# lfalive/fast-genomic-data-processing

Hardware: AMD Instinct MI355X
Metric: PairHMM GCUPS (higher is better)
Workload: dtype f32

## Files before the change

### fast-genomic-data-processing_amd/csrc/mgx_pairhmm.hip

```cpp
#include <hip/hip_runtime.h>

#include <algorithm>
#include <atomic>
#include <cerrno>
#include <cmath>
#include <cstdarg>
#include <cstdio>
#include <cstdlib>
#include <cstring>
#include <chrono>
#include <memory>
#include <mutex>
#include <new>
#include <thread>
#include <string>
#include <vector>

#include "../../include/mgx_pairhmm.h"
#include "mgx_common.h"
#include "mgx_tables.h"
#include "pairhmm_pack.h"
#include "pairhmm_kernels.hip.inc"

using mgx::set_error;
// ... 2 lines not shown

constexpr int kNarrowMaxRPL = 8, kG8MaxRPL = 8, kG16MaxRPL = 12, kG64MinRPL = 4, kG64MaxRPL = 16;
constexpr int kMaxRowsG4 = 4 * kNarrowMaxRPL, kMaxRowsG8 = 8 * kG8MaxRPL;
constexpr int kMaxRowsG16 = 16 * kG16MaxRPL;
constexpr int kMaxRowsG64 = 64 * kG64MaxRPL;
constexpr int kMaxRowsStrip = 1 << 20;
constexpr int kStripMarkRPL = kG64MaxRPL + 1;
constexpr uint32_t kMaxLdsPerBlock = 64 * 1024;

struct Bin {
    int G = 0, RPL = 0;
    int Gd = 0, RPLd = 0;
    uint32_t job_begin = 0, job_count = 0;
    uint32_t max_h = 0;
    uint64_t cells = 0, alg_bytes = 0;
    uint32_t block = 256, lds_stride = 0, grid_f32 = 0, grid_f64 = 0, grid_f64_all = 0;
    bool strip = false;
};


struct Slab {
    uint8_t* dev = nullptr;
    uint8_t* pin = nullptr;
    size_t cap = 0, pin_cap = 0;
};
constexpr size_t kStageLimit = 256u << 20;
constexpr size_t kMaxEventSets = 64;
constexpr size_t kMinSlab = 1u << 20;
}

struct mgx_pairhmm {
// ... 10 lines not shown
    int n_cu = 256;
    std::vector<Slab> free_slabs;
    void* d_strip = nullptr; size_t strip_cap = 0;
};

struct mgx_pairhmm_batch {
    uint64_t n_pairs = 0;
    std::vector<Bin> bins;
    Slab slab;
    size_t in_bytes = 0, o_out = 0, o_used = 0, result_bytes = 0;
    uint8_t *d_bases = nullptr, *d_qual = nullptr, *d_ins = nullptr, *d_del = nullptr,
            *d_gcp = nullptr, *d_hap = nullptr, *d_used = nullptr;
    Job* d_jobs = nullptr;
    uint32_t* d_rerun_list = nullptr;
    uint32_t* d_rerun_count = nullptr;
    double* d_out = nullptr;
    std::vector<Job> host_jobs;
    bool has_model = false;
    uint32_t n_reads = 0;
    uint64_t* d_read_len = nullptr;
    uint8_t* d_keep = nullptr;
    uint32_t *d_row_off = nullptr, *d_row_nh = nullptr;
    size_t o_keep = 0;
    double log10_rate = 0, max_err = 0;
    hipEvent_t uploaded = nullptr;
    std::vector<hipEvent_t> ev;
    std::vector<uint64_t> acct_cells, acct_bytes;
    std::vector<int8_t> acct_multi;
    uint32_t ev_sets = 0;
    uint32_t runs_timed = 0;
// ... 26 lines not shown
    HIP_TRY(hipMalloc((void**)dst, bytes));
    if (src) HIP_TRY(hipMemcpyAsync(*dst, src, bytes, hipMemcpyHostToDevice, s));
    return 0;
}

inline void shape_of(uint32_t R, int* G, int* RPL) {
    static const int min_g = [] { const char* e = getenv("MGX_PAIRHMM_MIN_G"); const int v = e ? atoi(e) : 4; return v; }();
    const uint32_t g8_rows = (uint32_t)kMaxRowsG8;
    if (R <= (uint32_t)kMaxRowsG4 && min_g <= 4) { *G = 4; *RPL = (int)((R + 3) / 4); }
    else if (R <= g8_rows && min_g <= 8) { *G = 8; *RPL = (int)((R + 7) / 8); }
    else if (R <= (uint32_t)kMaxRowsG16) { *G = 16; *RPL = (int)((R + 15) / 16); }
    else if (R <= (uint32_t)kMaxRowsG64) { *G = 64; *RPL = std::max(kG64MinRPL, (int)((R + 63) / 64)); }
    else if (R <= (uint32_t)kMaxRowsStrip) { *G = 64; *RPL = kStripMarkRPL; }
    else { *G = 0; *RPL = 0; }
}
inline uint32_t lds_bytes(const Bin& bin, bool f32) {
    const uint32_t waves = bin.block / 64u, groups = bin.block / (uint32_t)(f32 ? bin.G : bin.Gd);
    const uint32_t etab = f32 ? (uint32_t)((bin.RPL + 1) / 2) * kNumCodes * 512u : 0u;
    return waves * etab + groups * bin.lds_stride;
}
constexpr int kBinG8 = kNarrowMaxRPL, kBinG16 = kBinG8 + kG8MaxRPL, kBinG64 = kBinG16 + kG16MaxRPL;
constexpr int kBinStrip = kBinG64 + (kG64MaxRPL - kG64MinRPL + 1);
constexpr int kBins = kBinStrip + 1;
inline int bin_index(int G, int RPL) {
    if (G == 64 && RPL == kStripMarkRPL) return kBinStrip;
    return G == 4 ? RPL - 1 : G == 8 ? kBinG8 + RPL - 1 : G == 16 ? kBinG16 + RPL - 1 : kBinG64 + RPL - kG64MinRPL;
}
inline void bin_shape(int k, Bin* b) {
    if (k == kBinStrip) { b->G = 64; b->RPL = kG64MaxRPL; b->Gd = 64; b->RPLd = kG64MaxRPL; b->strip = true; return; }
    if (k < kBinG8) { b->G = 4; b->RPL = k + 1; }
    else if (k < kBinG16) { b->G = 8; b->RPL = k - kBinG8 + 1; }
    else if (k < kBinG64) { b->G = 16; b->RPL = k - kBinG16 + 1; }
    else { b->G = 64; b->RPL = k - kBinG64 + kG64MinRPL; }
    if (b->G == 16 && b->RPL > 8) { b->Gd = 64; b->RPLd = (16 * b->RPL + 63) / 64; }
    else { b->Gd = b->G; b->RPLd = b->RPL; }
}
constexpr uint64_t kMergeBelow = 4096;

int finalize_bin(Bin& bin, int n_cu) {
    bin.lds_stride = (bin.max_h + 2u * (uint32_t)std::max(bin.G, bin.Gd) + 8u + 15u) & ~15u;
    bin.block = 64;
    if (const char* e = getenv("MGX_PAIRHMM_BLOCK")) { const int v = atoi(e); if (v == 64 || v == 128 || v == 256) bin.block = (uint32_t)v; }
    while (bin.block > 64u && lds_bytes(bin, true) > kMaxLdsPerBlock) bin.block /= 2;
    if (lds_bytes(bin, true) > 160u * 1024u) {
        set_error("haplotype of %u bases does not fit the LDS staging buffer", bin.max_h);
        return -E2BIG;
    }
    if (bin.strip) {
        bin.block = 64;
        bin.grid_f32 = bin.grid_f64 = bin.grid_f64_all = std::min<uint32_t>(bin.job_count, (uint32_t)n_cu * 4u);
        return 0;
    }
    const uint32_t gpb = bin.block / bin.G, gpbd = bin.block / bin.Gd;
    bin.grid_f32 = (bin.job_count + gpb - 1) / gpb;
    bin.grid_f64_all = (bin.job_count + gpbd - 1) / gpbd;
    bin.grid_f64 = std::min<uint32_t>(bin.grid_f64_all, (uint32_t)n_cu * 8u);
    return 0;
}
void merge_small_bins(uint64_t (&count)[kBins], int (&remap)[kBins]) {
    for (int k = 0; k < kBins; ++k) remap[k] = k;
    for (int k = 0; k + 1 < kBins; ++k) {
        if (k + 1 == kBinG8 || k + 1 == kBinG16 || k + 1 == kBinG64 || k + 1 == kBinStrip) continue;
        if (count[k] && count[k] < kMergeBelow) { count[k + 1] += count[k]; count[k] = 0; remap[k] = k + 1; }
    }
    for (int k = 0; k < kBins; ++k) { int t = k; while (remap[t] != t) t = remap[t]; remap[k] = t; }
}

inline size_t align_up(size_t x, size_t a = 256) { return (x + a - 1) / a * a; }

int acquire_slab(mgx_pairhmm* c, size_t bytes, size_t pin_bytes, Slab* out) {
    int best = -1;
// ... 137 lines not shown
    release_slab(c, b->slab);
    if (b->uploaded) (void)hipEventDestroy(b->uploaded);
    if (b->done) (void)hipEventDestroy(b->done);
    for (auto e : b->ev) (void)hipEventDestroy(e);
    delete b;
}

namespace {

struct SlabLayout {
    uint64_t n = 0, n_reads = 0, n_haps = 0, n_regions = 0, read_bytes = 0, hap_bytes = 0;
    bool cross = false, model = false;
    size_t rtab = 0, rreg = 0, rpre = 0, gtab = 0, htab = 0;
    size_t jobs = 0, bases = 0, qual = 0, ins = 0, del = 0, gcp = 0, hap = 0;
    size_t mapq = 0, rlen = 0, roff = 0, rnh = 0;
    size_t rlist = 0, rcount = 0;
    size_t pin_bytes = 0;
    bool staged = true;
};

int lay_out_slab(mgx_pairhmm* c, bool always_stage, SlabLayout* L, mgx_pairhmm_batch* b) {
    size_t off = 0;
    auto take = [&off](size_t bytes) { const size_t at = off; off = align_up(off + bytes); return at; };
    const uint64_t n = L->n, per_read = L->model ? L->n_reads : 0;
    if (L->cross) {
        L->rtab = take(L->n_reads * sizeof(SeqRef));
        L->rreg = take(L->n_reads * sizeof(uint32_t));
        L->rpre = take((L->n_reads + 1) * sizeof(uint32_t));
        L->gtab = take(L->n_regions * sizeof(RegionRef));
        L->htab = take(L->n_haps * sizeof(SeqRef));
    } else {
// ... 5 lines not shown
    L->del = take(L->read_bytes);
    L->gcp = take(L->read_bytes);
    L->hap = take(L->hap_bytes);
    L->mapq = take(per_read);
    L->rlen = take(per_read * sizeof(uint64_t));
    L->roff = take(per_read * sizeof(uint32_t));
    L->rnh = take(per_read * sizeof(uint32_t));
    b->in_bytes = off;
    b->o_out = take(n * sizeof(double));
    b->o_used = take(n);
    b->o_keep = take(per_read);
    b->result_bytes = off - b->o_out;
    L->pin_bytes = off;
    if (L->cross) L->jobs = take(n * sizeof(Job));
    L->rlist = take(2 * n * sizeof(uint32_t));
    L->rcount = take(64 * sizeof(uint32_t));
    L->staged = always_stage || L->pin_bytes <= kStageLimit;
    if (const int rc = acquire_slab(c, off, L->staged ? L->pin_bytes : 0, &b->slab)) return rc;
    uint8_t* dv = b->slab.dev;
    b->d_jobs = (Job*)(dv + L->jobs);
    b->d_bases = dv + L->bases; b->d_qual = dv + L->qual; b->d_ins = dv + L->ins; b->d_del = dv + L->del;
    b->d_gcp = dv + L->gcp; b->d_hap = dv + L->hap;
    b->d_out = (double*)(dv + b->o_out); b->d_used = dv + b->o_used;
    b->d_rerun_list = (uint32_t*)(dv + L->rlist); b->d_rerun_count = (uint32_t*)(dv + L->rcount);
    if (L->model) {
        b->d_read_len = (uint64_t*)(dv + L->rlen); b->d_keep = dv + b->o_keep;
        b->d_row_off = (uint32_t*)(dv + L->roff); b->d_row_nh = (uint32_t*)(dv + L->rnh);
    }
    return 0;
}

ReadModel make_read_model(const mgx_read_model_t& model) {
    ReadModel rm{};
    rm.rate_factor = model.pcr_rate_factor; rm.bq_threshold = model.base_quality_threshold;
    rm.constant_gcp = model.constant_gcp;
    for (int i = 0; i <= 20; ++i) {
        const double d = 40.0 - std::exp((double)i / ((double)std::max(rm.rate_factor, 1) * M_PI));
        const int v = (d > 0.0 ? (int)(d + 0.5) : (int)(d - 0.5)) + 1;
        rm.pcr_cache[i] = (uint8_t)(char)std::max(10, v);
// ... 349 lines not shown
    mgx_pairhmm_batch* b = r.b;
    if (!r.timing) return 0;
    if (b->ev.empty()) {
        const size_t per = b->bins.size() * 4;
        b->ev_sets = (uint32_t)std::max<size_t>(1, std::min<size_t>(kMaxEventSets, 1024 / per));
        b->ev.resize(per * b->ev_sets);
        for (auto& e : b->ev) HIP_TRY(hipEventCreate(&e));
    }
    r.ev = b->ev.data() + (size_t)(b->runs_timed % b->ev_sets) * b->bins.size() * 4;
    return 0;
}

int begin_run(Run& r) {
    mgx_pairhmm* c = r.c; mgx_pairhmm_batch* b = r.b;
    if (b->uploaded) HIP_TRY(hipStreamWaitEvent(r.s, b->uploaded, 0));
    HIP_TRY(hipMemsetAsync(b->d_rerun_count, 0, 64 * sizeof(uint32_t), r.s));
    HIP_TRY(hipMemsetAsync(b->d_used, 0, b->n_pairs, r.s));
    r.n_str = (int)std::min<size_t>((size_t)c->n_streams, b->bins.size());
    if (r.n_str > 1) {
        HIP_TRY(hipEventRecord(c->ev_fork, r.s));
        for (int q = 0; q + 1 < r.n_str; ++q) HIP_TRY(hipStreamWaitEvent(c->aux[q], c->ev_fork, 0));
    }
    KernelArgs& base = r.base;
    base.jobs = b->d_jobs;
    base.bases = b->d_bases; base.qual = b->d_qual; base.ins = b->d_ins; base.del = b->d_del;
    base.gcp = b->d_gcp; base.hap_bases = b->d_hap;
    base.out_log10 = b->d_out; base.used_f64 = b->d_used;
    base.log10_initial_f = c->log10_initial_f;
    base.log10_initial_d = c->log10_initial_d;
    return 0;
}

void survey_narrow(Run& r) {
    const std::vector<Bin>& bins = r.b->bins;
    r.first_narrow = bins.size();
    for (size_t k = 0; k < bins.size(); ++k) {
        const Bin& bn = bins[k];
        if (!is_narrow(bn)) continue;
        if (r.first_narrow == bins.size()) r.first_narrow = k;
        r.n_narrow_jobs = std::max(r.n_narrow_jobs, bn.job_begin + bn.job_count);
        r.narrow_max_h = std::max(r.narrow_max_h, bn.max_h);
        r.narrow_rows = std::max(r.narrow_rows, (uint32_t)(bn.G * bn.RPL));
// ... 17 lines not shown
        return bx.RPL != by.RPL ? bx.RPL > by.RPL : bx.G > by.G;
    });
    MultiArgs m{};
    m.a = r.base;
    m.a.rerun_list = b->d_rerun_list; m.a.rerun_count = b->d_rerun_count + kSharedCount;
    m.a.job_list = nullptr; m.a.n_dyn = nullptr;
    m.a.ph2pr = c->d_ph2pr_f; m.a.mm = c->d_mm_f; m.a.ph2pr_div3 = c->d_div3_f; m.a.gap_ratio = c->d_ratio_f;
    m.n_bins = (uint32_t)set.size();
    uint32_t blocks = 0, lds = 0;
    size_t book = set[0];
    uint64_t cells = 0, bytes = 0;
    for (size_t q = 0; q < set.size(); ++q) {
        const Bin& bn = b->bins[set[q]];
        m.block_first[q] = blocks; blocks += bn.grid_f32;
        m.job_first[q] = bn.job_begin; m.job_count[q] = bn.job_count; m.lds_stride[q] = bn.lds_stride;
        m.G[q] = (uint8_t)bn.G; m.RPL[q] = (uint8_t)bn.RPL;
        lds = std::max(lds, lds_bytes(bn, true));
        if (bn.cells > b->bins[book].cells) book = set[q];
        cells += bn.cells; bytes += bn.alg_bytes;
        r.in_multi[set[q]] = 1;
        b->acct_cells[set[q]] = 0; b->acct_bytes[set[q]] = 0;
    }
    m.block_first[set.size()] = blocks;
    b->acct_cells[book] = cells; b->acct_bytes[book] = bytes; b->acct_multi[book] = (int8_t)(1 + gset);
    if (r.timing) for (size_t q : set) if (q != book) { HIP_TRY(hipEventRecord(r.ev[4 * q + 0], r.s)); HIP_TRY(hipEventRecord(r.ev[4 * q + 1], r.s)); }
    if (r.timing) HIP_TRY(hipEventRecord(r.ev[4 * book + 0], r.s));
    if (gset == 0) hipLaunchKernelGGL(pairhmm_fwd_multi<0>, dim3(blocks), dim3(64), lds, r.s, m);
    else           hipLaunchKernelGGL(pairhmm_fwd_multi<1>, dim3(blocks), dim3(64), lds, r.s, m);
    if (r.timing) HIP_TRY(hipEventRecord(r.ev[4 * book + 1], r.s));
    return 0;
}

// ... 20 lines not shown
int launch_class(Run& r, size_t k, hipStream_t sk) {
    mgx_pairhmm* c = r.c; mgx_pairhmm_batch* b = r.b;
    hipEvent_t* ev = r.ev;
    const Bin& bin = b->bins[k];
    const bool shared = is_narrow(bin) && !r.force_f64;
    KernelArgs a = r.base;
    if (bin.strip) {
        a.strip_stride = (bin.max_h + 63u) & ~63u;
        if (const int rc = ensure_strip_scratch(c, (size_t)bin.grid_f32 * 6u * a.strip_stride * sizeof(double))) return rc;
        a.strip_scratch = c->d_strip;
    }
    a.rerun_list = shared ? b->d_rerun_list : b->d_rerun_list + bin.job_begin;
    a.rerun_count = b->d_rerun_count + (shared ? kSharedCount : (int)k);
    a.lds_stride = bin.lds_stride;
    a.job_first = bin.job_begin;
    if (!r.force_f64 && !r.in_multi[k]) {
        a.job_list = nullptr; a.n_dyn = nullptr; a.n_static = bin.job_count;
        a.ph2pr = c->d_ph2pr_f; a.mm = c->d_mm_f; a.ph2pr_div3 = c->d_div3_f; a.gap_ratio = c->d_ratio_f;
        KernelFn f = bin.strip ? (KernelFn)pairhmm_fwd_strip<float> : pick_kernel<float>(bin.G, bin.RPL);
        if (!f) { set_error("no fp32 kernel for G=%d RPL=%d", bin.G, bin.RPL); return -ENOSYS; }
        if (r.timing) HIP_TRY(hipEventRecord(ev[4 * k + 0], sk));
        hipLaunchKernelGGL(f, dim3(bin.grid_f32), dim3(bin.block), lds_bytes(bin, true), sk, a);
        if (r.timing) HIP_TRY(hipEventRecord(ev[4 * k + 1], sk));
    }
    const bool books_shared = shared && k == r.first_narrow;
    if (r.timing && !books_shared) HIP_TRY(hipEventRecord(ev[4 * k + 2], sk));
    if (!shared) {
        if (r.force_f64) { a.job_list = nullptr; a.n_dyn = nullptr; a.n_static = bin.job_count; }
        else { a.job_list = a.rerun_list; a.n_dyn = a.rerun_count; a.n_static = 0; }
        const int rc = launch_f64(r, a, bin.Gd, bin.RPLd, r.force_f64 ? bin.grid_f64_all : bin.grid_f64, bin.block, lds_bytes(bin, false), sk);
        if (rc) return rc;
    }
    if (r.timing && !books_shared) HIP_TRY(hipEventRecord(ev[4 * k + 3], sk));
    return 0;
}

int launch_classes(Run& r) {
    mgx_pairhmm* c = r.c; mgx_pairhmm_batch* b = r.b;
    std::vector<size_t> order(b->bins.size());
    for (size_t k = 0; k < order.size(); ++k) order[k] = k;
    std::stable_sort(order.begin(), order.end(), [&](size_t x, size_t y) { return b->bins[x].cells > b->bins[y].cells; });
    for (size_t at = 0; at < order.size(); ++at) {
        hipStream_t sk = (int)(at % (size_t)r.n_str) == 0 ? r.s : c->aux[at % (size_t)r.n_str - 1];
        if (const int rc = launch_class(r, order[at], sk)) return rc;
    }
    for (int q = 0; q + 1 < r.n_str; ++q) {
        HIP_TRY(hipEventRecord(c->ev_join[q], c->aux[q]));
        HIP_TRY(hipStreamWaitEvent(r.s, c->ev_join[q], 0));
    }
    return 0;
}

int launch_shared_f64(Run& r) {
    if (!r.n_narrow_jobs || r.force_f64) return 0;
    KernelArgs a = r.base;
    a.job_list = r.b->d_rerun_list; a.n_dyn = r.b->d_rerun_count + kSharedCount; a.n_static = 0; a.job_first = 0;
    a.lds_stride = (r.narrow_max_h + 2u * 16u + 8u + 15u) & ~15u;
    const int RPLd = (int)((r.narrow_rows + 15) / 16);
// ... 60 lines not shown
    if (!c) { set_error("ctx is NULL"); return -EINVAL; }
    HIP_TRY(hipSetDevice(c->device));
    HIP_TRY(hipStreamSynchronize(c->compute));
    return 0;
}

int mgx_pairhmm_batch_stats(mgx_pairhmm_t* c, mgx_pairhmm_batch_t* b, mgx_pairhmm_stats_t* out) {
    if (!c || !b || !out) { set_error("NULL argument"); return -EINVAL; }
    HIP_TRY(hipSetDevice(c->device));
    HIP_TRY(hipStreamSynchronize(c->compute));
    mgx_pairhmm_stats_t st = b->stats;
    const bool force_f64 = (c->flags & MGX_PAIRHMM_FORCE_DOUBLE) != 0;
    st.n_launches_f32 = force_f64 ? 0 : (uint32_t)b->bins.size();
    st.n_launches_f64 = (uint32_t)b->bins.size();
    st.n_rerun_f64 = 0;
    if (b->ran && b->n_pairs) {
        std::vector<uint32_t> cnt(64);
        HIP_TRY(hipMemcpy(cnt.data(), b->d_rerun_count, 64 * sizeof(uint32_t), hipMemcpyDeviceToHost));
        for (size_t k = 0; k < b->bins.size(); ++k) st.n_rerun_f64 += force_f64 ? b->bins[k].job_count : cnt[k];
        if (!force_f64) st.n_rerun_f64 += cnt[63];
        st.n_exact = cnt[62];
    }
    st.ms_f32 = st.ms_f64 = st.ms_f32_dominant = 0;
    st.dominant_cells = st.dominant_alg_bytes = 0;
    st.dominant_kernel[0] = 0;
    st.n_runs_timed = 0;
    if ((c->flags & MGX_PAIRHMM_TIMING) && b->ran && !b->ev.empty() && b->runs_timed) {
        const uint32_t n_sets = std::min(b->runs_timed, b->ev_sets);
        const bool acct = b->acct_cells.size() == b->bins.size();
        auto cells_of = [&](size_t k) { return acct ? b->acct_cells[k] : b->bins[k].cells; };
        size_t dom = 0;
        for (size_t k = 0; k < b->bins.size(); ++k) if (cells_of(k) >= cells_of(dom)) dom = k;
        double f32 = 0, f64 = 0, domms = 0;
// ... 387 lines not shown
```

### fast-genomic-data-processing_amd/csrc/pairhmm_kernels.hip.inc

```

#include <type_traits>

namespace {

struct Job {
    uint64_t read_off;
    uint64_t hap_off;
    uint32_t R;
    uint32_t H;
    uint32_t pair;
    uint32_t pad_;
};
static_assert(sizeof(Job) == 32, "Job is 32 bytes");

struct KernelArgs {
    const Job* jobs;
    const uint32_t* job_list;
    const uint32_t* n_dyn;
    uint32_t n_static;
    uint32_t job_first;
    const uint8_t* bases;
    const uint8_t* qual;
    const uint8_t* ins;
    const uint8_t* del;
    const uint8_t* gcp;
    const uint8_t* hap_bases;
    const void* ph2pr;
    const void* mm;
    const void* ph2pr_div3;
    const void* gap_ratio;
    double* out_log10;
    uint8_t* used_f64;
    uint32_t* rerun_list;
    uint32_t* rerun_count;
    uint32_t lds_stride;
    void* strip_scratch;
    uint32_t strip_stride;
    float log10_initial_f;
    double log10_initial_d;
};

constexpr double kExactBelow = 1e-280;
constexpr int kCodeN = 4;
constexpr int kCodePad = 7;

__device__ __forceinline__ int base_code(int b) {
    int c = 0;
    c = (b == 'C') ? 1 : c;
    c = (b == 'T') ? 2 : c;
// ... 41 lines not shown
    const int src = (j == G - 1) ? lane : lane + S;
    return __shfl(v, src, 64);
}

__device__ __forceinline__ float fma_(float a, float b, float c) { return __builtin_fmaf(a, b, c); }
__device__ __forceinline__ double fma_(double a, double b, double c) { return __builtin_fma(a, b, c); }

template <typename T> struct Prec;
template <> struct Prec<float> {
    static __device__ __forceinline__ float initial() { return 0x1p120f; }
};
template <> struct Prec<double> {
    static __device__ __forceinline__ double initial() { return 0x1p1020; }
};

#ifndef MGX_PAIRHMM_CODES
#define MGX_PAIRHMM_CODES 5
#endif
constexpr int kNumCodes = MGX_PAIRHMM_CODES;
template <int RPL> constexpr int etab_bytes_per_wave() { return ((RPL + 1) / 2) * kNumCodes * 64 * 8; }

template <typename T, int G, int RPL, bool STRIP = false, bool EXACT = false>
__device__ __forceinline__ void pairhmm_body(const KernelArgs& a, uint8_t* smem, const uint32_t block, const uint32_t n_blocks) {
    constexpr int GPW = 64 / G;
    constexpr bool kETab = (sizeof(T) == 4);
    constexpr bool kSix = (sizeof(T) == 4) && !EXACT;
    constexpr int RP2 = (RPL + 1) / 2;
    constexpr int S = lane_stride<G>();
    const int gpb = (int)blockDim.x / G;
    const int tid = (int)threadIdx.x;
    const int lane = tid & 63;
    const int wave = tid >> 6;
    const int j = G < 16 ? (lane & 15) / S : lane % G;
    const int grp = wave * GPW + (G < 16 ? (lane >> 4) * S + (lane & 15) % S : lane / G);
    const int n_waves = (int)blockDim.x >> 6;
    uint8_t* etab = smem + (kETab ? (size_t)wave * etab_bytes_per_wave<RPL>() : 0);
    uint8_t* hapbuf = smem + (kETab ? (size_t)n_waves * etab_bytes_per_wave<RPL>() : 0) +
                      (size_t)grp * a.lds_stride;
    const T* __restrict__ ph2pr = (const T*)a.ph2pr;
    const T* __restrict__ mm = (const T*)a.mm;
    const T* __restrict__ ph2pr_div3 = (const T*)a.ph2pr_div3;
    const T* __restrict__ gap_ratio = (const T*)a.gap_ratio;
    const uint32_t n_jobs = a.n_dyn ? *a.n_dyn : a.n_static;

    for (uint32_t base = block * (uint32_t)gpb; base < n_jobs; base += n_blocks * (uint32_t)gpb) {
        const uint32_t slot = base + (uint32_t)grp;
        const bool live = slot < n_jobs;
        uint32_t job_idx = 0;
        Job job;
        job.read_off = 0; job.hap_off = 0; job.R = 0; job.H = 0; job.pair = 0; job.pad_ = 0;
        if (live) {
            job_idx = a.job_list ? a.job_list[slot] : a.job_first + slot;
// ... 95 lines not shown
                    rb[s] = code;
                }
            }
        }
        if constexpr (kETab) {
            float* et = reinterpret_cast<float*>(etab) + lane * 2;
#pragma unroll
            for (int s = 0; s < RPL; ++s)
#pragma unroll
                for (int code = 0; code < kNumCodes; ++code)
                    et[((s >> 1) * kNumCodes + code) * 128 + (s & 1)] =
                        (code == rb[s] || code == kCodeN) ? eM[s] : eX[s];
        }
        __syncthreads();

        const int nsteps_g = live ? (H + nl - 1) : 0;
        int nmax = nsteps_g, nmin = live ? nsteps_g : 0x7fffffff;
        if constexpr (GPW > 1) {
#pragma unroll
            for (int off = 1; off < 64; off <<= 1) {
                if (off >= S && off < (G < 16 ? 16 : G)) continue;
                const int o1 = __shfl_xor(nmax, off, 64), o2 = __shfl_xor(nmin, off, 64);
                nmax = o1 > nmax ? o1 : nmax;
                nmin = o2 < nmin ? o2 : nmin;
            }
        }
        nmax = __builtin_amdgcn_readfirstlane(nmax);
        nmin = __builtin_amdgcn_readfirstlane(nmin);
        if (nmin > nmax) nmin = nmax;

        const uint8_t* hp_lane = hapbuf + (G - j);
        const uint8_t* et_lane = etab + lane * 8;
// ... 63 lines not shown
                }
                y_above = SIX ? init_y : g_own[0] * init_y;
            }
            const T old_y = (j == 0) ? y_above : (T)0;
            T uaM = 0, uaX = 0, uaY = old_y, ubM = 0, ubX = 0, ubY = old_y;
            if constexpr (STRIP) {
                if (strip > 0) {
                    uaY = 0; ubY = 0;
                    if (j == 0 && H > 0) { ubM = bprev[0]; ubX = bprev[a.strip_stride]; ubY = bprev[2u * a.strip_stride]; }
                }
            }

            auto column = [&](const T (&ec)[RPL], T& o2M, T& o2X, T& o2Y, const T o1M, const T o1X, bool count, const int dcol) {
                T Mn[RPL], Xn[RPL], Yn[RPL];
                if constexpr (SIX) {
                    Mn[0] = fma_(k3[0], o2Y, fma_(o2M, k0[0], o2X)) * ec[0];
                    Xn[0] = fma_(o1X, k2[0], o1M * k1[0]);
                    Yn[0] = fma_(py[0], k4[0], pm[0]);
#pragma unroll
                    for (int s = 1; s < RPL; ++s) {
                        Mn[s] = fma_(k3[s], py[s - 1], fma_(pm[s - 1], k0[s], px[s - 1])) * ec[s];
                        Xn[s] = fma_(Xn[s - 1], k2[s], Mn[s - 1] * k1[s]);
                        Yn[s] = fma_(py[s], k4[s], pm[s]);
                    }
                } else if constexpr (SC) {
                    Mn[0] = (fma_(o2M, k0[0], o2X) + o2Y) * ec[0];
                    Xn[0] = fma_(o1X, k2[0], o1M * k1[0]);
                    Yn[0] = fma_(py[0], k4[0], pm[0] * k3[0]);
#pragma unroll
                    for (int s = 1; s < RPL; ++s) {
                        Mn[s] = (fma_(pm[s - 1], k0[s], px[s - 1]) + py[s - 1]) * ec[s];
                        Xn[s] = fma_(Xn[s - 1], k2[s], Mn[s - 1] * k1[s]);
                        Yn[s] = fma_(py[s], k4[s], pm[s] * k3[s]);
                    }
                } else if constexpr (EXACT) {
                    Mn[0] = ((o2M * k0[0] + o2X * k1[0]) + o2Y * k1[0]) * ec[0];
                    Xn[0] = o1M * k2[0] + o1X * k3[0];
                    Yn[0] = pm[0] * k4[0] + py[0] * k3[0];
#pragma unroll
// ... 52 lines not shown
                t = uaM; uaM = ubM; ubM = t;
                t = uaX; uaX = ubX; ubX = t;
                t = uaY; uaY = ubY; ubY = t;
                load_e(hn, e);
            }
        };
        if constexpr (EXACT) sweep(std::integral_constant<int, kPlain>{});
        else if (use_plain) sweep(std::integral_constant<int, kPlain>{});
        else if constexpr (kSix) sweep(std::integral_constant<int, kSixOp>{});
        else sweep(std::integral_constant<int, kScaled>{});
      }

        if (live && j == nl - 1) {
            const T res = sumM + sumX;
            if constexpr (sizeof(T) == 4) {
                if (res < 1e-28f || group_hap_n) {
                    const uint32_t k = atomicAdd(a.rerun_count, 1u);
                    a.rerun_list[k] = job_idx;
                } else {
                    a.out_log10[job.pair] = (double)(log10f(res) - a.log10_initial_f);
                }
            } else {
                if (!EXACT && a.rerun_count && res < kExactBelow) {
                    const uint32_t k = atomicAdd(a.rerun_count, 1u);
                    a.rerun_list[k] = job_idx;
                } else {
                    a.out_log10[job.pair] = log10(res) - a.log10_initial_d;
                    a.used_f64[job.pair] = 1;
                }
            }
        }
    }
}

template <typename T, int G, int RPL>
#ifndef MGX_HMM_MINWAVES_8
#define MGX_HMM_MINWAVES_8 4
#endif
__global__ __launch_bounds__(256, (sizeof(T) == 4 && RPL == 7) ? MGX_HMM_MINWAVES_8 : (sizeof(T) == 4 && RPL == 10) ? 3 : 1) void pairhmm_fwd(KernelArgs a) {
    extern __shared__ __attribute__((aligned(16))) uint8_t smem[];
    pairhmm_body<T, G, RPL>(a, smem, blockIdx.x, gridDim.x);
}

constexpr int kStripG = 64, kStripRPL = 16;
template <typename T>
__global__ __launch_bounds__(64) void pairhmm_fwd_strip(KernelArgs a) {
    extern __shared__ __attribute__((aligned(16))) uint8_t smem[];
    pairhmm_body<T, kStripG, kStripRPL, true>(a, smem, blockIdx.x, gridDim.x);
}
__global__ __launch_bounds__(64) void pairhmm_fwd_exact(KernelArgs a) {
    extern __shared__ __attribute__((aligned(16))) uint8_t smem[];
    pairhmm_body<double, kStripG, kStripRPL, true, true>(a, smem, blockIdx.x, gridDim.x);
}

constexpr int kMultiBins = 16;
struct MultiArgs {
    KernelArgs a;
    uint32_t n_bins;
    uint32_t block_first[kMultiBins + 1];
    uint32_t job_first[kMultiBins], job_count[kMultiBins], lds_stride[kMultiBins];
    uint8_t G[kMultiBins], RPL[kMultiBins];
};

template <int GSET>
__device__ __forceinline__ void pairhmm_multi_body(const MultiArgs& m, uint8_t* smem) {
    uint32_t k = 0;
    while (k + 1 < m.n_bins && blockIdx.x >= m.block_first[k + 1]) ++k;
    KernelArgs a = m.a;
    a.job_first = m.job_first[k]; a.n_static = m.job_count[k]; a.lds_stride = m.lds_stride[k];
    const uint32_t blk = blockIdx.x - m.block_first[k], nblk = m.block_first[k + 1] - m.block_first[k];
    const int code = (int)m.G[k] * 16 + (int)m.RPL[k];
#define MGX_MCASE(g, r) case (g) * 16 + (r): pairhmm_body<float, g, r>(a, smem, blk, nblk); break;
    if constexpr (GSET == 0) {
        switch (code) {
            MGX_MCASE(16, 1) MGX_MCASE(16, 2) MGX_MCASE(16, 3) MGX_MCASE(16, 4) MGX_MCASE(16, 5) MGX_MCASE(16, 6) MGX_MCASE(16, 7) MGX_MCASE(16, 8)
            default: break;
        }
    } else {
        switch (code) {
            MGX_MCASE(8, 1) MGX_MCASE(8, 2) MGX_MCASE(8, 3) MGX_MCASE(8, 4) MGX_MCASE(8, 5) MGX_MCASE(8, 6) MGX_MCASE(8, 7) MGX_MCASE(8, 8)
            MGX_MCASE(4, 1) MGX_MCASE(4, 2) MGX_MCASE(4, 3) MGX_MCASE(4, 4) MGX_MCASE(4, 5) MGX_MCASE(4, 6) MGX_MCASE(4, 7) MGX_MCASE(4, 8)
            default: break;
        }
    }
#undef MGX_MCASE
}

// ... 123 lines not shown
    for (uint32_t h = lane; h < n_haps; h += 64) best = fmax(best, row[h]);
#pragma unroll
    for (int off = 32; off > 0; off >>= 1) best = fmax(best, __shfl_xor(best, off, 64));
    if (!__builtin_isinf(log10_rate) && n_haps > 1) {
        const double cap = best + log10_rate;
        for (uint32_t h = lane; h < n_haps; h += 64) if (row[h] < cap) row[h] = cap;
    }
    if (lane == 0) {
        const double max_err = fmin(2.0, ceil((double)read_len[r] * max_error_per_base));
        keep[r] = !(best < max_err * -4.0);
    }
}

using KernelFn = void (*)(KernelArgs);

template <typename T>
KernelFn pick_kernel(int G, int RPL) {
#define MGX_CASE(g, r) if (G == g && RPL == r) return pairhmm_fwd<T, g, r>;
    MGX_CASE(4, 1) MGX_CASE(4, 2) MGX_CASE(4, 3) MGX_CASE(4, 4) MGX_CASE(4, 5) MGX_CASE(4, 6) MGX_CASE(4, 7) MGX_CASE(4, 8)
    MGX_CASE(8, 1) MGX_CASE(8, 2) MGX_CASE(8, 3) MGX_CASE(8, 4) MGX_CASE(8, 5) MGX_CASE(8, 6) MGX_CASE(8, 7) MGX_CASE(8, 8)
    MGX_CASE(16, 1) MGX_CASE(16, 2) MGX_CASE(16, 3) MGX_CASE(16, 4)
    MGX_CASE(16, 5) MGX_CASE(16, 6) MGX_CASE(16, 7) MGX_CASE(16, 8)
    if constexpr (sizeof(T) == 4) { MGX_CASE(16, 9) MGX_CASE(16, 10) MGX_CASE(16, 11) MGX_CASE(16, 12) }
    if constexpr (sizeof(T) == 8) { MGX_CASE(64, 3) }
    MGX_CASE(64, 4) MGX_CASE(64, 5) MGX_CASE(64, 6) MGX_CASE(64, 7) MGX_CASE(64, 8)
    MGX_CASE(64, 9) MGX_CASE(64, 10) MGX_CASE(64, 11) MGX_CASE(64, 12)
    MGX_CASE(64, 13) MGX_CASE(64, 14) MGX_CASE(64, 15) MGX_CASE(64, 16)
#undef MGX_CASE
    return nullptr;
}

}
```

### fast-genomic-data-processing_amd/native.py

```python
import ctypes as C
import os

_HERE = os.path.dirname(os.path.abspath(__file__))
_LIB = None


class MgxError(RuntimeError):
    pass


def lib_path():
    return os.path.join(_HERE, "libmgx.so")


class PairHMMInput(C.Structure):
    _fields_ = [
        ("n_reads", C.c_uint64), ("read_off", C.c_void_p), ("bases", C.c_void_p),
        ("qual", C.c_void_p), ("ins", C.c_void_p), ("del_", C.c_void_p), ("gcp", C.c_void_p),
        ("n_haps", C.c_uint64), ("hap_off", C.c_void_p), ("hap_bases", C.c_void_p),
        ("n_pairs", C.c_uint64), ("pair_read", C.c_void_p), ("pair_hap", C.c_void_p),
    ]


class PairHMMStats(C.Structure):
    _fields_ = [
        ("n_pairs", C.c_uint64), ("cells", C.c_uint64), ("alg_bytes", C.c_uint64),
        ("n_rerun_f64", C.c_uint64), ("n_launches_f32", C.c_uint32), ("n_launches_f64", C.c_uint32),
        ("n_runs_timed", C.c_uint32), ("ms_f32", C.c_float), ("ms_f64", C.c_float), ("ms_f32_dominant", C.c_float),
        ("dominant_cells", C.c_uint64), ("dominant_alg_bytes", C.c_uint64),
        ("dominant_kernel", C.c_char * 64), ("n_exact", C.c_uint64),
    ]


class QueueConfig(C.Structure):
    _fields_ = [("n_devices", C.c_uint32), ("devices", C.c_void_p), ("lanes_per_device", C.c_uint32),
                ("depth", C.c_uint32), ("batch_pairs", C.c_uint32), ("flags", C.c_uint)]


class QueueStats(C.Structure):
    _fields_ = [("n_pairs", C.c_uint64), ("n_batches", C.c_uint64), ("cells", C.c_uint64),
                ("bytes_h2d", C.c_uint64), ("bytes_d2h", C.c_uint64), ("seconds", C.c_double),
                ("pack_seconds", C.c_double), ("wait_seconds", C.c_double), ("n_lanes", C.c_uint32),
                ("batches_per_device", C.c_uint64 * 16)]


# ... 178 lines not shown
```

### include/mgx_pairhmm.h

```cpp
#ifndef MGX_PAIRHMM_H
#define MGX_PAIRHMM_H

#include <stddef.h>
#include <stdint.h>

#ifdef __cplusplus
extern "C" {
#endif

typedef struct mgx_pairhmm mgx_pairhmm_t;
typedef struct mgx_pairhmm_batch mgx_pairhmm_batch_t;

#define MGX_PAIRHMM_FORCE_DOUBLE 1u
#define MGX_PAIRHMM_TIMING       2u
#define MGX_PAIRHMM_PACKED_FP32  4u
#define MGX_CU_PATTERN(p) (((unsigned)(p) & 0xFFu) << 8)
#define MGX_STREAM_HIGH_PRIORITY (1u << 16)

typedef struct mgx_pairhmm_input {
    uint64_t n_reads;
    const uint64_t* read_off;
    const uint8_t* bases;
    const uint8_t* qual;
    const uint8_t* ins;
// ... 10 lines not shown
typedef struct mgx_pairhmm_stats {
    uint64_t n_pairs;
    uint64_t cells;
    uint64_t alg_bytes;
    uint64_t n_rerun_f64;
    uint32_t n_launches_f32;
    uint32_t n_launches_f64;
    uint32_t n_runs_timed;
    float ms_f32;
    float ms_f64;
    float ms_f32_dominant;
    uint64_t dominant_cells;
    uint64_t dominant_alg_bytes;
    char dominant_kernel[64];
    uint64_t n_exact;
} mgx_pairhmm_stats_t;

const char* mgx_last_error(void);

#define MGX_DEVICE_AUTO (-1)

int mgx_pairhmm_create(int device, unsigned flags, mgx_pairhmm_t** out);
void mgx_pairhmm_destroy(mgx_pairhmm_t* ctx);

int mgx_pairhmm_compute(mgx_pairhmm_t* ctx, const mgx_pairhmm_input_t* in, double* out_log10);

int mgx_pairhmm_compute_regions(mgx_pairhmm_t* ctx, uint32_t n_regions, const mgx_pairhmm_input_t* regions,
                                double* const* out_log10);

int mgx_pairhmm_batch_create(mgx_pairhmm_t* ctx, const mgx_pairhmm_input_t* in,
// ... 61 lines not shown
```

Before: 6346.

## Split N-containing haplotype jobs into a separate five-code fp32 kernel pass

The main fp32 kernels now use a four-code emission table, which shrinks LDS per wave. Groups whose haplotype contains N are skipped and appended to a new per-bin list instead of being sent to the fp64 rerun path. A second dynamic-list fp32 launch with five codes then processes those jobs. The SIX column recurrence is also reordered to update the prior-state arrays in place, and bins in the multi-bin launch are forced onto the main stream. Cost: an extra launch per bin, more counters, and a stats struct ABI change.

```diff
diff --git a/fast-genomic-data-processing_amd/csrc/mgx_pairhmm.hip b/fast-genomic-data-processing_amd/csrc/mgx_pairhmm.hip
--- a/fast-genomic-data-processing_amd/csrc/mgx_pairhmm.hip
+++ b/fast-genomic-data-processing_amd/csrc/mgx_pairhmm.hip
@@ -40,7 +40,7 @@
     uint32_t job_begin = 0, job_count = 0;
     uint32_t max_h = 0;
     uint64_t cells = 0, alg_bytes = 0;
-    uint32_t block = 256, lds_stride = 0, grid_f32 = 0, grid_f64 = 0, grid_f64_all = 0;
+    uint32_t block = 256, lds_stride = 0, grid_f32 = 0, grid_f64 = 0, grid_f64_all = 0, grid_nhap = 0;
     bool strip = false;
 };
 
@@ -81,6 +81,7 @@
     Job* d_jobs = nullptr;
     uint32_t* d_rerun_list = nullptr;
     uint32_t* d_rerun_count = nullptr;
+    uint32_t* d_nhap_list = nullptr;
     double* d_out = nullptr;
     std::vector<Job> host_jobs;
     bool has_model = false;
@@ -137,9 +138,9 @@
     else if (R <= (uint32_t)kMaxRowsStrip) { *G = 64; *RPL = kStripMarkRPL; }
     else { *G = 0; *RPL = 0; }
 }
-inline uint32_t lds_bytes(const Bin& bin, bool f32) {
+inline uint32_t lds_bytes(const Bin& bin, bool f32, int codes = kMaxCodes) {
     const uint32_t waves = bin.block / 64u, groups = bin.block / (uint32_t)(f32 ? bin.G : bin.Gd);
-    const uint32_t etab = f32 ? (uint32_t)((bin.RPL + 1) / 2) * kNumCodes * 512u : 0u;
+    const uint32_t etab = f32 ? (uint32_t)((bin.RPL + 1) / 2) * (uint32_t)codes * 512u : 0u;
     return waves * etab + groups * bin.lds_stride;
 }
 constexpr int kBinG8 = kNarrowMaxRPL, kBinG16 = kBinG8 + kG8MaxRPL, kBinG64 = kBinG16 + kG16MaxRPL;
@@ -159,6 +160,8 @@
     else { b->Gd = b->G; b->RPLd = b->RPL; }
 }
 constexpr uint64_t kMergeBelow = 4096;
+constexpr int kNhapCount = 64, kCounters = 128;
+static_assert(kBins <= 62 && kNhapCount + kBins <= kCounters, "counter slots");
 
 int finalize_bin(Bin& bin, int n_cu) {
     bin.lds_stride = (bin.max_h + 2u * (uint32_t)std::max(bin.G, bin.Gd) + 8u + 15u) & ~15u;
@@ -178,6 +181,7 @@
     bin.grid_f32 = (bin.job_count + gpb - 1) / gpb;
     bin.grid_f64_all = (bin.job_count + gpbd - 1) / gpbd;
     bin.grid_f64 = std::min<uint32_t>(bin.grid_f64_all, (uint32_t)n_cu * 8u);
+    bin.grid_nhap = std::min<uint32_t>(bin.grid_f32, (uint32_t)n_cu * 8u);
     return 0;
 }
 void merge_small_bins(uint64_t (&count)[kBins], int (&remap)[kBins]) {
@@ -345,7 +349,7 @@
     size_t rtab = 0, rreg = 0, rpre = 0, gtab = 0, htab = 0;
     size_t jobs = 0, bases = 0, qual = 0, ins = 0, del = 0, gcp = 0, hap = 0;
     size_t mapq = 0, rlen = 0, roff = 0, rnh = 0;
-    size_t rlist = 0, rcount = 0;
+    size_t rlist = 0, nlist = 0, rcount = 0;
     size_t pin_bytes = 0;
     bool staged = true;
 };
@@ -381,7 +385,8 @@
     L->pin_bytes = off;
     if (L->cross) L->jobs = take(n * sizeof(Job));
     L->rlist = take(2 * n * sizeof(uint32_t));
-    L->rcount = take(64 * sizeof(uint32_t));
+    L->nlist = take(n * sizeof(uint32_t));
+    L->rcount = take(kCounters * sizeof(uint32_t));
     L->staged = always_stage || L->pin_bytes <= kStageLimit;
     if (const int rc = acquire_slab(c, off, L->staged ? L->pin_bytes : 0, &b->slab)) return rc;
     uint8_t* dv = b->slab.dev;
@@ -390,6 +395,7 @@
     b->d_gcp = dv + L->gcp; b->d_hap = dv + L->hap;
     b->d_out = (double*)(dv + b->o_out); b->d_used = dv + b->o_used;
     b->d_rerun_list = (uint32_t*)(dv + L->rlist); b->d_rerun_count = (uint32_t*)(dv + L->rcount);
+    b->d_nhap_list = (uint32_t*)(dv + L->nlist);
     if (L->model) {
         b->d_read_len = (uint64_t*)(dv + L->rlen); b->d_keep = dv + b->o_keep;
         b->d_row_off = (uint32_t*)(dv + L->roff); b->d_row_nh = (uint32_t*)(dv + L->rnh);
@@ -769,7 +775,7 @@
 int begin_run(Run& r) {
     mgx_pairhmm* c = r.c; mgx_pairhmm_batch* b = r.b;
     if (b->uploaded) HIP_TRY(hipStreamWaitEvent(r.s, b->uploaded, 0));
-    HIP_TRY(hipMemsetAsync(b->d_rerun_count, 0, 64 * sizeof(uint32_t), r.s));
+    HIP_TRY(hipMemsetAsync(b->d_rerun_count, 0, kCounters * sizeof(uint32_t), r.s));
     HIP_TRY(hipMemsetAsync(b->d_used, 0, b->n_pairs, r.s));
     r.n_str = (int)std::min<size_t>((size_t)c->n_streams, b->bins.size());
     if (r.n_str > 1) {
@@ -781,6 +787,7 @@
     base.bases = b->d_bases; base.qual = b->d_qual; base.ins = b->d_ins; base.del = b->d_del;
     base.gcp = b->d_gcp; base.hap_bases = b->d_hap;
     base.out_log10 = b->d_out; base.used_f64 = b->d_used;
+    base.nhap_list = b->d_nhap_list; base.nhap_count = b->d_rerun_count + kNhapCount;
     base.log10_initial_f = c->log10_initial_f;
     base.log10_initial_d = c->log10_initial_d;
     return 0;
@@ -828,8 +835,8 @@
         const Bin& bn = b->bins[set[q]];
         m.block_first[q] = blocks; blocks += bn.grid_f32;
         m.job_first[q] = bn.job_begin; m.job_count[q] = bn.job_count; m.lds_stride[q] = bn.lds_stride;
-        m.G[q] = (uint8_t)bn.G; m.RPL[q] = (uint8_t)bn.RPL;
-        lds = std::max(lds, lds_bytes(bn, true));
+        m.G[q] = (uint8_t)bn.G; m.RPL[q] = (uint8_t)bn.RPL; m.bin[q] = (uint8_t)set[q];
+        lds = std::max(lds, lds_bytes(bn, true, 4));
         if (bn.cells > b->bins[book].cells) book = set[q];
         cells += bn.cells; bytes += bn.alg_bytes;
         r.in_multi[set[q]] = 1;
@@ -880,14 +887,25 @@
     a.rerun_count = b->d_rerun_count + (shared ? kSharedCount : (int)k);
     a.lds_stride = bin.lds_stride;
     a.job_first = bin.job_begin;
-    if (!r.force_f64 && !r.in_multi[k]) {
-        a.job_list = nullptr; a.n_dyn = nullptr; a.n_static = bin.job_count;
+    a.nhap_list = b->d_nhap_list + bin.job_begin;
+    a.nhap_count = b->d_rerun_count + kNhapCount + (int)k;
+    if (!r.force_f64) {
         a.ph2pr = c->d_ph2pr_f; a.mm = c->d_mm_f; a.ph2pr_div3 = c->d_div3_f; a.gap_ratio = c->d_ratio_f;
-        KernelFn f = bin.strip ? (KernelFn)pairhmm_fwd_strip<float> : pick_kernel<float>(bin.G, bin.RPL);
-        if (!f) { set_error("no fp32 kernel for G=%d RPL=%d", bin.G, bin.RPL); return -ENOSYS; }
-        if (r.timing) HIP_TRY(hipEventRecord(ev[4 * k + 0], sk));
-        hipLaunchKernelGGL(f, dim3(bin.grid_f32), dim3(bin.block), lds_bytes(bin, true), sk, a);
-        if (r.timing) HIP_TRY(hipEventRecord(ev[4 * k + 1], sk));
+        const bool first = !r.in_multi[k];
+        if (first) {
+            a.job_list = nullptr; a.n_dyn = nullptr; a.n_static = bin.job_count;
+            KernelFn f = bin.strip ? (KernelFn)pairhmm_fwd_strip<float> : pick_kernel<float, 4>(bin.G, bin.RPL);
+            if (!f) { set_error("no fp32 kernel for G=%d RPL=%d", bin.G, bin.RPL); return -ENOSYS; }
+            if (r.timing) HIP_TRY(hipEventRecord(ev[4 * k + 0], sk));
+            hipLaunchKernelGGL(f, dim3(bin.grid_f32), dim3(bin.block), lds_bytes(bin, true, bin.strip ? kMaxCodes : 4), sk, a);
+        }
+        if (!bin.strip) {
+            KernelFn f5 = pick_kernel<float, kMaxCodes>(bin.G, bin.RPL);
+            if (!f5) { set_error("no fp32 kernel for G=%d RPL=%d", bin.G, bin.RPL); return -ENOSYS; }
+            a.job_list = a.nhap_list; a.n_dyn = a.nhap_count; a.n_static = 0;
+            hipLaunchKernelGGL(f5, dim3(bin.grid_nhap), dim3(bin.block), lds_bytes(bin, true, kMaxCodes), sk, a);
+        }
+        if (r.timing && first) HIP_TRY(hipEventRecord(ev[4 * k + 1], sk));
     }
     const bool books_shared = shared && k == r.first_narrow;
     if (r.timing && !books_shared) HIP_TRY(hipEventRecord(ev[4 * k + 2], sk));
@@ -908,6 +926,7 @@
     std::stable_sort(order.begin(), order.end(), [&](size_t x, size_t y) { return b->bins[x].cells > b->bins[y].cells; });
     for (size_t at = 0; at < order.size(); ++at) {
         hipStream_t sk = (int)(at % (size_t)r.n_str) == 0 ? r.s : c->aux[at % (size_t)r.n_str - 1];
+        if (r.in_multi[order[at]]) sk = r.s;
         if (const int rc = launch_class(r, order[at], sk)) return rc;
     }
     for (int q = 0; q + 1 < r.n_str; ++q) {
@@ -998,9 +1017,11 @@
     st.n_launches_f32 = force_f64 ? 0 : (uint32_t)b->bins.size();
     st.n_launches_f64 = (uint32_t)b->bins.size();
     st.n_rerun_f64 = 0;
+    st.n_nhap_f32 = 0;
     if (b->ran && b->n_pairs) {
-        std::vector<uint32_t> cnt(64);
-        HIP_TRY(hipMemcpy(cnt.data(), b->d_rerun_count, 64 * sizeof(uint32_t), hipMemcpyDeviceToHost));
+        std::vector<uint32_t> cnt(kCounters);
+        HIP_TRY(hipMemcpy(cnt.data(), b->d_rerun_count, kCounters * sizeof(uint32_t), hipMemcpyDeviceToHost));
+        for (size_t k = 0; k < b->bins.size(); ++k) st.n_nhap_f32 += cnt[kNhapCount + k];
         for (size_t k = 0; k < b->bins.size(); ++k) st.n_rerun_f64 += force_f64 ? b->bins[k].job_count : cnt[k];
         if (!force_f64) st.n_rerun_f64 += cnt[63];
         st.n_exact = cnt[62];
diff --git a/fast-genomic-data-processing_amd/csrc/pairhmm_kernels.hip.inc b/fast-genomic-data-processing_amd/csrc/pairhmm_kernels.hip.inc
--- a/fast-genomic-data-processing_amd/csrc/pairhmm_kernels.hip.inc
+++ b/fast-genomic-data-processing_amd/csrc/pairhmm_kernels.hip.inc
@@ -33,6 +33,8 @@
     uint8_t* used_f64;
     uint32_t* rerun_list;
     uint32_t* rerun_count;
+    uint32_t* nhap_list;
+    uint32_t* nhap_count;
     uint32_t lds_stride;
     void* strip_scratch;
     uint32_t strip_stride;
@@ -104,16 +106,16 @@
     static __device__ __forceinline__ double initial() { return 0x1p1020; }
 };
 
-#ifndef MGX_PAIRHMM_CODES
-#define MGX_PAIRHMM_CODES 5
-#endif
-constexpr int kNumCodes = MGX_PAIRHMM_CODES;
-template <int RPL> constexpr int etab_bytes_per_wave() { return ((RPL + 1) / 2) * kNumCodes * 64 * 8; }
-
-template <typename T, int G, int RPL, bool STRIP = false, bool EXACT = false>
+constexpr int kMaxCodes = 5;
+template <int RPL, int CODES> constexpr int etab_bytes_per_wave() { return ((RPL + 1) / 2) * CODES * 64 * 8; }
+
+template <typename T, int G, int RPL, bool STRIP = false, bool EXACT = false, int CODES = kMaxCodes>
 __device__ __forceinline__ void pairhmm_body(const KernelArgs& a, uint8_t* smem, const uint32_t block, const uint32_t n_blocks) {
     constexpr int GPW = 64 / G;
     constexpr bool kETab = (sizeof(T) == 4);
+    constexpr int kNumCodes = CODES;
+    static_assert(CODES == 4 || CODES == kMaxCodes, "four or five code columns");
+    static_assert(kETab || CODES == kMaxCodes, "fp64 has no table: the N code is compared");
     constexpr bool kSix = (sizeof(T) == 4) && !EXACT;
     constexpr int RP2 = (RPL + 1) / 2;
     constexpr int S = lane_stride<G>();
@@ -124,8 +126,8 @@
     const int j = G < 16 ? (lane & 15) / S : lane % G;
     const int grp = wave * GPW + (G < 16 ? (lane >> 4) * S + (lane & 15) % S : lane / G);
     const int n_waves = (int)blockDim.x >> 6;
-    uint8_t* etab = smem + (kETab ? (size_t)wave * etab_bytes_per_wave<RPL>() : 0);
-    uint8_t* hapbuf = smem + (kETab ? (size_t)n_waves * etab_bytes_per_wave<RPL>() : 0) +
+    uint8_t* etab = smem + (kETab ? (size_t)wave * etab_bytes_per_wave<RPL, CODES>() : 0);
+    uint8_t* hapbuf = smem + (kETab ? (size_t)n_waves * etab_bytes_per_wave<RPL, CODES>() : 0) +
                       (size_t)grp * a.lds_stride;
     const T* __restrict__ ph2pr = (const T*)a.ph2pr;
     const T* __restrict__ mm = (const T*)a.mm;
@@ -251,8 +253,9 @@
         }
         __syncthreads();
 
-        const int nsteps_g = live ? (H + nl - 1) : 0;
-        int nmax = nsteps_g, nmin = live ? nsteps_g : 0x7fffffff;
+        const bool swept = live && !group_hap_n;
+        const int nsteps_g = swept ? (H + nl - 1) : 0;
+        int nmax = nsteps_g, nmin = swept ? nsteps_g : 0x7fffffff;
         if constexpr (GPW > 1) {
 #pragma unroll
             for (int off = 1; off < 64; off <<= 1) {
@@ -346,15 +349,18 @@
             auto column = [&](const T (&ec)[RPL], T& o2M, T& o2X, T& o2Y, const T o1M, const T o1X, bool count, const int dcol) {
                 T Mn[RPL], Xn[RPL], Yn[RPL];
                 if constexpr (SIX) {
-                    Mn[0] = fma_(k3[0], o2Y, fma_(o2M, k0[0], o2X)) * ec[0];
-                    Xn[0] = fma_(o1X, k2[0], o1M * k1[0]);
-                    Yn[0] = fma_(py[0], k4[0], pm[0]);
-#pragma unroll
-                    for (int s = 1; s < RPL; ++s) {
-                        Mn[s] = fma_(k3[s], py[s - 1], fma_(pm[s - 1], k0[s], px[s - 1])) * ec[s];
-                        Xn[s] = fma_(Xn[s - 1], k2[s], Mn[s - 1] * k1[s]);
-                        Yn[s] = fma_(py[s], k4[s], pm[s]);
-                    }
+#pragma unroll
+                    for (int s = RPL - 1; s >= 0; --s) {
+                        const T t = s ? fma_(k3[s], py[s - 1], fma_(pm[s - 1], k0[s], px[s - 1]))
+                                      : fma_(k3[0], o2Y, fma_(o2M, k0[0], o2X));
+                        py[s] = fma_(py[s], k4[s], pm[s]);
+                        pm[s] = t * ec[s];
+                    }
+                    px[0] = fma_(o1X, k2[0], o1M * k1[0]);
+#pragma unroll
+                    for (int s = 1; s < RPL; ++s) px[s] = fma_(px[s - 1], k2[s], pm[s - 1] * k1[s]);
+#pragma unroll
+                    for (int s = 0; s < RPL; ++s) { Mn[s] = pm[s]; Xn[s] = px[s]; Yn[s] = py[s]; }
                 } else if constexpr (SC) {
                     Mn[0] = (fma_(o2M, k0[0], o2X) + o2Y) * ec[0];
                     Xn[0] = fma_(o1X, k2[0], o1M * k1[0]);
@@ -437,7 +443,10 @@
         if (live && j == nl - 1) {
             const T res = sumM + sumX;
             if constexpr (sizeof(T) == 4) {
-                if (res < 1e-28f || group_hap_n) {
+                if (group_hap_n) {
+                    const uint32_t k = atomicAdd(a.nhap_count, 1u);
+                    a.nhap_list[k] = job_idx;
+                } else if (res < 1e-28f) {
                     const uint32_t k = atomicAdd(a.rerun_count, 1u);
                     a.rerun_list[k] = job_idx;
                 } else {
@@ -456,13 +465,13 @@
     }
 }
 
-template <typename T, int G, int RPL>
+template <typename T, int G, int RPL, int CODES = kMaxCodes>
 #ifndef MGX_HMM_MINWAVES_8
 #define MGX_HMM_MINWAVES_8 4
 #endif
 __global__ __launch_bounds__(256, (sizeof(T) == 4 && RPL == 7) ? MGX_HMM_MINWAVES_8 : (sizeof(T) == 4 && RPL == 10) ? 3 : 1) void pairhmm_fwd(KernelArgs a) {
     extern __shared__ __attribute__((aligned(16))) uint8_t smem[];
-    pairhmm_body<T, G, RPL>(a, smem, blockIdx.x, gridDim.x);
+    pairhmm_body<T, G, RPL, false, false, CODES>(a, smem, blockIdx.x, gridDim.x);
 }
 
 constexpr int kStripG = 64, kStripRPL = 16;
@@ -483,6 +492,7 @@
     uint32_t block_first[kMultiBins + 1];
     uint32_t job_first[kMultiBins], job_count[kMultiBins], lds_stride[kMultiBins];
     uint8_t G[kMultiBins], RPL[kMultiBins];
+    uint8_t bin[kMultiBins];
 };
 
 template <int GSET>
@@ -491,9 +501,10 @@
     while (k + 1 < m.n_bins && blockIdx.x >= m.block_first[k + 1]) ++k;
     KernelArgs a = m.a;
     a.job_first = m.job_first[k]; a.n_static = m.job_count[k]; a.lds_stride = m.lds_stride[k];
+    a.nhap_list += m.job_first[k]; a.nhap_count += m.bin[k];
     const uint32_t blk = blockIdx.x - m.block_first[k], nblk = m.block_first[k + 1] - m.block_first[k];
     const int code = (int)m.G[k] * 16 + (int)m.RPL[k];
-#define MGX_MCASE(g, r) case (g) * 16 + (r): pairhmm_body<float, g, r>(a, smem, blk, nblk); break;
+#define MGX_MCASE(g, r) case (g) * 16 + (r): pairhmm_body<float, g, r, false, false, 4>(a, smem, blk, nblk); break;
     if constexpr (GSET == 0) {
         switch (code) {
             MGX_MCASE(16, 1) MGX_MCASE(16, 2) MGX_MCASE(16, 3) MGX_MCASE(16, 4) MGX_MCASE(16, 5) MGX_MCASE(16, 6) MGX_MCASE(16, 7) MGX_MCASE(16, 8)
@@ -647,9 +658,9 @@
 
 using KernelFn = void (*)(KernelArgs);
 
-template <typename T>
+template <typename T, int CODES = kMaxCodes>
 KernelFn pick_kernel(int G, int RPL) {
-#define MGX_CASE(g, r) if (G == g && RPL == r) return pairhmm_fwd<T, g, r>;
+#define MGX_CASE(g, r) if (G == g && RPL == r) return pairhmm_fwd<T, g, r, CODES>;
     MGX_CASE(4, 1) MGX_CASE(4, 2) MGX_CASE(4, 3) MGX_CASE(4, 4) MGX_CASE(4, 5) MGX_CASE(4, 6) MGX_CASE(4, 7) MGX_CASE(4, 8)
     MGX_CASE(8, 1) MGX_CASE(8, 2) MGX_CASE(8, 3) MGX_CASE(8, 4) MGX_CASE(8, 5) MGX_CASE(8, 6) MGX_CASE(8, 7) MGX_CASE(8, 8)
     MGX_CASE(16, 1) MGX_CASE(16, 2) MGX_CASE(16, 3) MGX_CASE(16, 4)
diff --git a/fast-genomic-data-processing_amd/native.py b/fast-genomic-data-processing_amd/native.py
--- a/fast-genomic-data-processing_amd/native.py
+++ b/fast-genomic-data-processing_amd/native.py
@@ -29,6 +29,7 @@
         ("n_runs_timed", C.c_uint32), ("ms_f32", C.c_float), ("ms_f64", C.c_float), ("ms_f32_dominant", C.c_float),
         ("dominant_cells", C.c_uint64), ("dominant_alg_bytes", C.c_uint64),
         ("dominant_kernel", C.c_char * 64), ("n_exact", C.c_uint64),
+        ("n_nhap_f32", C.c_uint64),
     ]
 
 
diff --git a/include/mgx_pairhmm.h b/include/mgx_pairhmm.h
--- a/include/mgx_pairhmm.h
+++ b/include/mgx_pairhmm.h
@@ -48,6 +48,7 @@
     uint64_t dominant_alg_bytes;
     char dominant_kernel[64];
     uint64_t n_exact;
+    uint64_t n_nhap_f32;
 } mgx_pairhmm_stats_t;
 
 const char* mgx_last_error(void);
```

Measured after the change: 6666, median of 6. 5.0% higher.
